# ethereum/c-kzg-4844

Hardware: AMD Instinct MI355X
Metric: blob_to_kzg_commitment throughput (higher is better)
Workload: dtype u32

## Files before the change

### c-kzg-4844_amd/csrc/device.hpp

```cpp
#pragma once
#include <vector>
#include <hip/hip_runtime.h>
#include <atomic>
#include <chrono>
#include <cstdint>
#include <cstdio>
#include <cstdlib>
#include <ctime>
#include <sys/syscall.h>
#include <unistd.h>
#include "g1.hpp"

namespace ckzg {
namespace dev {

constexpr int N_BLOB = 4096;
constexpr int N_EXT = 8192;
constexpr int N_CELL = 64;
constexpr int N_CELLS_EXT = 128;


#ifdef CKZG_AB
static inline long ab_knob(const char *env, long dflt) {
    const char *e = getenv(env);
// ... 93 lines not shown
    for (;;) {
        e = query();
        if (e != hipErrorNotReady) break;
        const int64_t waited = note.waited_us();
        if (waited < spin_us || (waited >= spin_from && waited <= spin_to)) continue;
        if (note.expired()) {
            int d = -1;
            if (hipGetDevice(&d) == hipSuccess && d >= 0 && d < 64) wedged_devices_ref().fetch_or((uint64_t)1 << d, std::memory_order_relaxed);
            (void)hipGetLastError();
            return hipErrorLaunchTimeOut;
        }
        if (div <= 0) continue;
        int64_t step = waited / div;
        step = step < 20 ? 20 : (step > 1000 ? 1000 : step);
        if (waited < spin_from && waited + step > spin_from) step = spin_from - waited;
        sleep_us(step < 5 ? 5 : step);
    }
    last = note.waited_us();
    (void)hipGetLastError();
    return e;
}
inline hipError_t sync_stream(hipStream_t s, int64_t spin_us = 100) {
    return bounded_device_wait([s]() { return hipStreamQuery(s); }, "stream", (const void *)s, spin_us);
}
inline hipError_t sync_event(hipEvent_t ev, int64_t spin_us = 100) {
    return bounded_device_wait([ev]() { return hipEventQuery(ev); }, "event", (const void *)ev, spin_us);
}
inline hipError_t ensure_event(hipEvent_t &e) {
    if (e) return hipSuccess;
    const hipError_t r = hipEventCreateWithFlags(&e, hipEventDisableTiming);
    if (r != hipSuccess) e = nullptr;
    return r;
}

inline std::atomic<int> g_poison_byte{0};
inline int poison_byte() { return g_poison_byte.load(std::memory_order_relaxed); }
inline hipError_t poison_fill(void *p, size_t bytes, hipStream_t s, int byte) {
    if (!p || !bytes) return hipSuccess;
    const hipError_t e = hipMemsetAsync(p, byte, bytes, s);
    return e != hipSuccess ? e : sync_stream(s);
}
inline hipError_t poison_fresh(void *p, size_t bytes, hipStream_t s) {
    const int b = poison_byte();
    return b ? poison_fill(p, bytes, s, b) : hipSuccess;
}

struct FixedBaseTable {
    G1Affine *d_table = nullptr;
    int npoints = 0;
    int wbits = 0;
    int nwin = 0;
    int twin = 0;
    size_t half = 0;
    size_t bytes() const { return (size_t)twin * npoints * half * sizeof(G1Affine); }
    static int twin_for(int wbits) { return 127 / wbits + 1; }
};

struct Scratch {
    void *ptr = nullptr;
    size_t cap = 0;
};

inline double &reserve_scale() {
    static thread_local double s = 1.0;
    return s;
}
struct ReserveScale {
    double old;
    ReserveScale(size_t max_units, size_t n) : old(reserve_scale()) {
        const double f = n ? (double)max_units / (double)n : 1.0;
        reserve_scale() = f < 1.0 ? 1.0 : f;
    }
    ~ReserveScale() { reserve_scale() = old; }
    ReserveScale(const ReserveScale &) = delete;
    ReserveScale &operator=(const ReserveScale &) = delete;
};
inline size_t reserve_scaled(size_t bytes) {
    const double f = reserve_scale();
    if (f <= 1.0) return bytes;
    const double want = (double)bytes * f, cap = (double)bytes + (double)((size_t)1 << 30);
    return (size_t)(want < cap ? want : cap);
}
inline size_t speculative_bytes(size_t need, size_t ahead) {
    if (ahead <= need) return need;
    size_t free_b = 0, total_b = 0;
    if (hipMemGetInfo(&free_b, &total_b) != hipSuccess) {
        (void)hipGetLastError();
        return need;
    }
    return ahead <= free_b / 8 ? ahead : need;
}

struct Arena {
    void *base = nullptr;
    size_t cap = 0, used = 0;
    hipStream_t stream = nullptr;
    bool begin(size_t bytes) {
        bytes += 64 * 256;
        used = 0;
        if (cap >= bytes) return true;
        const size_t old_cap = cap;
        if (base) (void)hipFree(base);
        base = nullptr;
        cap = 0;
        const size_t slack = (bytes >> 1) < ((size_t)256 << 20) ? (bytes >> 1) : ((size_t)256 << 20);
        size_t want = bytes + slack;
// ... 262 lines not shown
```

### c-kzg-4844_amd/csrc/f30_test_ops.hpp

```cpp
#pragma once
#include "g1_30.hpp"

#define CKZG_F30_TEST_OPS                                                                                          \
    OP_MUL(1, 1) OP_MUL(5, 1) OP_MUL(4, 1) OP_MUL(17, 18)                                                          \
    OP_SQR(5) OP_SQR(2) OP_SQR(17)                                                                                 \
    OP_MUL_ADD2(2, 5, 1, 1) OP_MUL_ADD2(17, 17, 5, 5)                                                              \
    OP_NORM(1, 1) OP_NORM(2, 5) OP_NORM(2, 2) OP_NORM(2, 4) OP_NORM(3, 3) OP_NORM(3, 200)                          \
    OP_ADD(1, 1, 1, 1) OP_ADD(1, 1, 2, 2) OP_SUB(1, 1, 1, 4) OP_SUB(1, 1, 1, 3)                                    \
    OP_NEG(1) OP_UNPACK() OP_TO_F28() OP_CONST()

namespace ckzg {
namespace f30test {

constexpr int STATE_WORDS = 52;
constexpr int ENTRY_WORDS = 24;
constexpr int EXIT_WORDS = 56;

template <int L, int V>
HD F30<L, V> ld(const int32_t *p) {
    F30<L, V> r;
#pragma unroll
    for (int j = 0; j < 13; j++) r.l[j] = p[j];
    return r;
}
// ... 45 lines not shown
#undef OP_NEG
#undef OP_UNPACK
#undef OP_TO_F28
#undef OP_CONST
    return false;
}

inline const char *desc() {
    return ""
#define OP_MUL(VA, VB) "mul " #VA " " #VB "\n"
#define OP_SQR(VA) "sqr " #VA "\n"
#define OP_MUL_ADD2(VA, VB, VC, VD) "mul_add2 " #VA " " #VB " " #VC " " #VD "\n"
#define OP_NORM(LA, VA) "norm " #LA " " #VA "\n"
#define OP_ADD(LA, VA, LB, VB) "add " #LA " " #VA " " #LB " " #VB "\n"
#define OP_SUB(LA, VA, LB, VB) "sub " #LA " " #VA " " #LB " " #VB "\n"
#define OP_NEG(V) "neg " #V "\n"
#define OP_UNPACK() "unpack\n"
#define OP_TO_F28() "to_f28\n"
#define OP_CONST() "const\n"
        CKZG_F30_TEST_OPS
#undef OP_MUL
#undef OP_SQR
#undef OP_MUL_ADD2
#undef OP_NORM
#undef OP_ADD
#undef OP_SUB
#undef OP_NEG
#undef OP_UNPACK
#undef OP_TO_F28
#undef OP_CONST
        ;
}

HD void ld_state(XYZZ30 &acc, const int32_t *s) {
    acc.x = ld<1, 4>(s);
    acc.w = ld<1, 1>(s + 13);
    acc.zz = ld<1, 1>(s + 26);
    acc.zzz = ld<1, 1>(s + 39);
}
HD void st_state(int32_t *o, const XYZZ30 &acc) {
#pragma unroll
    for (int j = 0; j < 13; j++) {
        o[j] = acc.x.l[j];
        o[13 + j] = acc.w.l[j];
        o[26 + j] = acc.zz.l[j];
        o[39 + j] = acc.zzz.l[j];
    }
}

HDNI inline void madd_step(int32_t *o, uint8_t *oflags, const int32_t *s, const uint8_t *flags, const uint32_t *entry) {
    XYZZ30 acc;
    ld_state(acc, s);
    bool inf = flags[0] != 0, yneg = flags[1] != 0;
    xyzz30_madd_alt(acc, inf, yneg, f30_unpack(entry), f30_unpack(entry + 12), flags[2] != 0);
    st_state(o, acc);
    oflags[0] = inf ? 1 : 0;
    oflags[1] = yneg ? 1 : 0;
}

HDNI inline void phi_step(int32_t *o, const int32_t *s) {
    XYZZ30 acc;
    ld_state(acc, s);
    xyzz30_apply_phi(acc);
    st_state(o, acc);
}

HDNI inline void exit_step(uint32_t *o, uint8_t *met, const int32_t *s) {
    XYZZ30 acc;
    ld_state(acc, s);
    const XYZZ28 r = xyzz30_to_xyzz28(acc);
#pragma unroll
    for (int j = 0; j < 14; j++) {
        o[j] = r.x.l[j];
        o[14 + j] = r.y.l[j];
        o[28 + j] = r.zz.l[j];
        o[42 + j] = r.zzz.l[j];
    }
    *met = xyzz30_met_equal_x(r) ? 1 : 0;
}

}
}
```

### c-kzg-4844_amd/csrc/fp30.hpp

```cpp
#pragma once
#include "fp28.hpp"

namespace ckzg {

#include "fp30_consts.inc"

template <int LB, int VB>
struct F30 {
    int32_t l[13];
};

HD int32_t f30_sext(uint32_t v) { return (int32_t)(v << 2) >> 2; }

HD void mad64s(int64_t &acc, int32_t a, int32_t b) { acc += (int64_t)a * b; }

HD int32_t f30_take_digit(int64_t &acc, int k) {
    if ((k & 1) != 0) acc += ((int64_t)1 << 29) + ((int64_t)1 << 59);
    const int32_t d = (int32_t)((uint32_t)acc & 0x3fffffffu) - (1 << 29);
    acc >>= 30;
    return d;
}

#if defined(__HIP_DEVICE_COMPILE__) && defined(CKZG_F28_ASM_BLOCKS)
#define CKZG_F30_USE_ASM_BLOCKS 1
#include "fp30_asm_cols.inc"
#endif

namespace f30detail {
constexpr int MAX_TERMS = 31;
}

template <int VA, int VB>
HD F30<1, 1> mul(const F30<1, VA> &a, const F30<1, VB> &b) {
    static_assert(13 + 13 + 2 <= f30detail::MAX_TERMS, "signed 64-bit column accumulator would overflow");
    static_assert(VA * VB <= 314, "Montgomery product would exceed p in magnitude");
#ifdef CKZG_F30_USE_ASM_BLOCKS
    {
        F30<1, 1> ra;
        f30asm_mul(ra.l, a.l, b.l);
        return ra;
    }
#endif
    int32_t q[13];
    int64_t acc = 0;
#pragma unroll
    for (int k = 0; k < 13; k++) {
#pragma unroll
        for (int i = 0; i <= k; i++) mad64s(acc, a.l[i], b.l[k - i]);
#pragma unroll
        for (int i = 0; i < k; i++) mad64s(acc, q[i], F30_P[k - i]);
        q[k] = f30_sext((uint32_t)acc * F30_NINV);
        mad64s(acc, q[k], F30_P[0]);
        acc >>= 30;
    }
    F30<1, 1> r;
#pragma unroll
    for (int k = 13; k < 25; k++) {
#pragma unroll
        for (int i = k - 12; i < 13; i++) mad64s(acc, a.l[i], b.l[k - i]);
#pragma unroll
        for (int i = k - 12; i < 13; i++) mad64s(acc, q[i], F30_P[k - i]);
        r.l[k - 13] = f30_take_digit(acc, k);
    }
    r.l[12] = (int32_t)acc;
    return r;
}

template <int VA, int VB, int VC, int VD>
HD F30<1, 1> mul_add2(const F30<1, VA> &a, const F30<1, VB> &b, const F30<1, VC> &c, const F30<1, VD> &d) {
    static_assert(3 * (F30_SPLIT_LO - 1 + 1) <= f30detail::MAX_TERMS && 3 * (25 - (F30_SPLIT_HI + 1)) <= f30detail::MAX_TERMS,
                  "an unsplit column would overflow");
// ... 74 lines not shown
    return r;
}

template <int LA, int VA, int LB, int VB>
HD F30<LA + LB, VA + VB> add(const F30<LA, VA> &a, const F30<LB, VB> &b) {
    static_assert(LA + LB <= 3, "limb would overflow 32 bits");
    F30<LA + LB, VA + VB> r;
#pragma unroll
    for (int j = 0; j < 13; j++) r.l[j] = a.l[j] + b.l[j];
    return r;
}

template <int LA, int VA, int LB, int VB>
HD F30<LA + LB, VA + VB> sub(const F30<LA, VA> &a, const F30<LB, VB> &b) {
    static_assert(LA + LB <= 3, "limb would overflow 32 bits");
    F30<LA + LB, VA + VB> r;
#pragma unroll
    for (int j = 0; j < 13; j++) r.l[j] = a.l[j] - b.l[j];
    return r;
}

template <int LA, int VA>
HD F30<1, VA> norm(const F30<LA, VA> &a) {
    static_assert(LA <= 3, "limb plus carry would overflow 32 bits");
    static_assert(VA <= 200, "top limb bound");
    F30<1, VA> r;
    int32_t c = 0;
#pragma unroll
    for (int j = 0; j < 12; j++) {
        const int32_t v = a.l[j] + c;
        r.l[j] = f30_sext((uint32_t)v);
        c = LA <= 2 ? (v - r.l[j]) >> 30 : (v >> 30) - (r.l[j] >> 31);
    }
    r.l[12] = a.l[12] + c;
    return r;
}

template <int V>
HD F30<1, V> f30_neg(const F30<1, V> &a) {
    F30<1, V> r;
#pragma unroll
    for (int j = 0; j < 13; j++) r.l[j] = -a.l[j];
    return r;
}

template <int V>
HD F30<1, V> f30_const(const int32_t (&c)[13]) {
    F30<1, V> r;
#pragma unroll
    for (int j = 0; j < 13; j++) r.l[j] = c[j];
    return r;
}

HD F30<1, 1> f30_unpack(const uint32_t *w) {
    F30<1, 1> r;
    uint32_t f[13];
#pragma unroll
    for (int j = 0; j < 13; j++) {
        const int bit = 30 * j, k = bit >> 5, sh = bit & 31;
        uint32_t lo = w[k] >> sh;
        if (sh > 2 && k + 1 < 12) lo |= w[k + 1] << (32 - sh);
        f[j] = lo;
    }
#pragma unroll
    for (int j = 0; j < 13; j++) {
        const int32_t s = j < 12 ? f30_sext(f[j]) : (int32_t)f[j];
        r.l[j] = j == 0 ? s : s + (int32_t)((f[j - 1] >> 29) & 1u);
    }
    return r;
}

HD F28<1, 2> f30_to_f28(const F30<1, 1> &a) {
    uint32_t f[13];
    int32_t c = 0;
#pragma unroll
    for (int j = 0; j < 12; j++) {
        const int32_t v = a.l[j] + F30_P[j] + c;
        f[j] = (uint32_t)v & 0x3fffffffu;
        c = v >> 30;
    }
    f[12] = (uint32_t)(a.l[12] + F30_P[12] + c);
    F28<1, 2> r;
#pragma unroll
    for (int j = 0; j < 14; j++) {
        const int bit = 28 * j, k = bit / 30, sh = bit - 30 * k;
        uint32_t lo = f[k] >> sh;
        if (sh > 2 && k + 1 < 13) lo |= f[k + 1] << (30 - sh);
        r.l[j] = j == 13 ? lo : (lo & M28);
    }
    return r;
}

}
```

### c-kzg-4844_amd/csrc/g1_30.hpp

```cpp
#pragma once
#include "fp30.hpp"
#include "g1_28.hpp"

namespace ckzg {

struct XYZZ30 {
    F30<1, 4> x;
    F30<1, 1> w;
    F30<1, 1> zz;
    F30<1, 1> zzz;
};

template <int V2, int V>
HD F30<1, V2> widen30(const F30<1, V> &a) {
    static_assert(V2 >= V, "bounds can only be loosened");
    F30<1, V2> r;
#pragma unroll
    for (int j = 0; j < 13; j++) r.l[j] = a.l[j];
    return r;
}

HD void xyzz30_madd_alt(XYZZ30 &acc, bool &inf, bool &yneg, const F30<1, 1> &x2, const F30<1, 1> &y2, bool dneg) {
    if (inf) yneg = false;
    const bool tneg = dneg != !yneg;
    const F30<1, 1> ny = f30_neg(y2);
    F30<1, 1> t;
#pragma unroll
    for (int j = 0; j < 13; j++) t.l[j] = tneg ? ny.l[j] : y2.l[j];
    if (inf) {
        acc.x = widen30<4>(mul(x2, f30_const<1>(F30_R392)));
        acc.w = mul(t, f30_const<1>(F30_R394));
        acc.zz = f30_const<1>(F30_R392);
        acc.zzz = f30_const<1>(F30_R394);
        inf = false;
        yneg = true;
        return;
    }
    auto u2 = mul(x2, acc.zz);
    auto tt = mul(t, acc.zzz);
    auto p = norm(sub(u2, acc.x));
    auto r = norm(add(tt, acc.w));
    auto pp = sqr(p);
    auto ppp = mul(p, pp);
    auto q = mul(acc.x, pp);
    auto rr = sqr(r);
    auto t1 = norm(add(ppp, add(q, q)));
    acc.x = norm(sub(rr, t1));
    auto d = norm(sub(q, acc.x));
    acc.w = mul_add2(r, d, acc.w, ppp);
    acc.zz = mul(acc.zz, pp);
    acc.zzz = mul(acc.zzz, ppp);
    yneg = !yneg;
}

HD void xyzz30_apply_phi(XYZZ30 &acc) { acc.x = widen30<4>(mul(acc.x, f30_const<1>(F30_BETA390))); }

HD XYZZ28 xyzz30_to_xyzz28(const XYZZ30 &acc) {
    XYZZ28 o;
    o.x = widen<1, 10>(f30_to_f28(mul(acc.x, f30_const<1>(F30_R392))));
    o.y = widen<1, 6>(f30_to_f28(mul(acc.w, f30_const<1>(F30_R392))));
    o.zz = f30_to_f28(mul(acc.zz, f30_const<1>(F30_R394)));
    o.zzz = f30_to_f28(mul(acc.zzz, f30_const<1>(F30_R394)));
    return o;
}

HD bool xyzz30_met_equal_x(const XYZZ28 &o) { return is_zero(o.zz); }

}
```

### c-kzg-4844_amd/csrc/msm.hip

```cpp
#include <chrono>
#include <cstring>
#include <vector>
#include "device.hpp"
#include "dev_inline.hpp"
#include "g1_28.hpp"
#include "g1_30.hpp"
#include "g1_quad.hpp"

namespace ckzg {
namespace dev {

int scratch_reserve(DeviceCtx *ctx, size_t bytes) {
    if (ctx->scratch.cap >= bytes) return 0;
    const size_t old_cap = ctx->scratch.cap;
    if (ctx->scratch.ptr) {
        HIP_TRY(dev::sync_stream(ctx->stream));
        HIP_TRY(hipFree(ctx->scratch.ptr));
        ctx->scratch.ptr = nullptr;
        ctx->scratch.cap = 0;
    }
    size_t want = bytes + (bytes >> 2);
    if (reserve_scaled(bytes) > want) want = reserve_scaled(bytes);
    if (old_cap) {
        const size_t step = old_cap < ((size_t)2 << 30) ? old_cap : ((size_t)2 << 30);
// ... 230 lines not shown
                tb_store_point(cur[k], x3, y3);
            }
        }
    }
}

int batch_to_affine_device(DeviceCtx *ctx, G1Affine *d_out, const G1XYZZ *d_in, Fp *d_prefix, size_t n) {
    if (n == 0) return 0;
    static const size_t solo_max = (size_t)ab_knob("CKZG_HIP_TO_AFFINE_SOLO_MAX", 4096);
    int L = n >= ((size_t)1 << 20) ? 128 : (n >= ((size_t)1 << 14) ? 16 : (n > solo_max ? 4 : 1));
    size_t threads = (n + L - 1) / L;
    hipLaunchKernelGGL(k_batch_to_affine, dim3((unsigned)((threads + 63) / 64)), dim3(64), 0, ctx->stream,
                       d_out, d_in, d_prefix, n, L, 0);
    HIP_TRY(hipGetLastError());
    return 0;
}


static int enqueue_affine_chain_table(hipStream_t stream, const FixedBaseTable &t, G1Affine *d_table, const G1XYZZ *d_wb,
                                      G1Affine *d_wba, Fp *d_prefix, const std::atomic<bool> *cancel) {
    const size_t nchains = (size_t)t.twin * t.npoints;
    {
        const int Lb = 16;
        const size_t th = (nchains + Lb - 1) / Lb;
        hipLaunchKernelGGL(k_batch_to_affine, dim3((unsigned)((th + 63) / 64)), dim3(64), 0, stream, d_wba, d_wb, d_prefix,
                           nchains, Lb, 1);
    }
    constexpr int LSEG = 8;
    const size_t entries = nchains * t.half;
    size_t seg = entries / ((size_t)262144 * LSEG);
    uint32_t seg2 = 16;
    while (seg2 < 512 && seg2 * 2 <= seg) seg2 *= 2;
    if (seg2 > t.half) seg2 = (uint32_t)t.half;
    const uint32_t nseg = (uint32_t)(t.half / seg2);
    const size_t chains_per_launch = cancel ? (size_t)4 * t.npoints : nchains;
    for (size_t c0 = 0; c0 < nchains; c0 += chains_per_launch) {
        if (cancel && cancel->load(std::memory_order_relaxed)) {
            (void)dev::sync_stream(stream);
            return 5;
        }
        if (cancel && c0) HIP_TRY(dev::sync_stream(stream));
        const size_t nc = nchains - c0 < chains_per_launch ? nchains - c0 : chains_per_launch;
        const size_t units = nc * nseg, threads = (units + LSEG - 1) / LSEG;
        hipLaunchKernelGGL(k_table_seeds, dim3((unsigned)((units + 63) / 64)), dim3(64), 0, stream, d_table + c0 * t.half,
                           d_wba + c0, (uint32_t)nc, (uint32_t)t.half, seg2);
        if (seg2 > 1)
            hipLaunchKernelGGL(k_table_steps<LSEG>, dim3((unsigned)((threads + 63) / 64)), dim3(64), 0, stream,
                               d_table + c0 * t.half, d_wba + c0, (uint32_t)nc, (uint32_t)t.half, seg2);
    }
    HIP_TRY(hipGetLastError());
    return 0;
}

int build_fixed_base_table(DeviceCtx *ctx, FixedBaseTable *t, const G1Affine *d_bases, int npoints,
                           int wbits, double *times_ms, const std::atomic<bool> *cancel) {
    if (wbits < 2 || wbits > 16) return 1;
    const auto t_start = std::chrono::steady_clock::now();
    t->npoints = npoints;
    t->wbits = wbits;
    t->twin = FixedBaseTable::twin_for(wbits);
    t->nwin = 2 * t->twin;
    t->half = (size_t)1 << (wbits - 1);
    DevTmp wb, prefix, table, wba;
    t->d_table = nullptr;
    HIP_TRY(hipMalloc(&table.p, t->bytes()));
    G1Affine *d_table = static_cast<G1Affine *>(table.p);
    HIP_TRY(hipMalloc(&wb.p, (size_t)t->twin * npoints * sizeof(G1XYZZ)));
    HIP_TRY(poison_fresh(wb.p, (size_t)t->twin * npoints * sizeof(G1XYZZ), ctx->stream));
    G1XYZZ *d_wb = static_cast<G1XYZZ *>(wb.p);
    const auto t_alloc = std::chrono::steady_clock::now();
    enqueue_window_bases(ctx->stream, d_wb, d_bases, npoints, wbits, t->twin);
    {
        const size_t nchains = (size_t)t->twin * npoints;
        HIP_TRY(hipMalloc(&wba.p, nchains * sizeof(G1Affine)));
        HIP_TRY(hipMalloc(&prefix.p, nchains * sizeof(Fp)));
        HIP_TRY(poison_fresh(wba.p, nchains * sizeof(G1Affine), ctx->stream));
        HIP_TRY(poison_fresh(prefix.p, nchains * sizeof(Fp), ctx->stream));
        int rc = enqueue_affine_chain_table(ctx->stream, *t, d_table, d_wb, static_cast<G1Affine *>(wba.p),
                                            static_cast<Fp *>(prefix.p), cancel);
        if (rc) return rc;
    }
    HIP_TRY(hipGetLastError());
    HIP_TRY(dev::sync_stream(ctx->stream));
    t->d_table = d_table;
    table.p = nullptr;
    if (times_ms) {
        const auto t_end = std::chrono::steady_clock::now();
        times_ms[0] += std::chrono::duration<double, std::milli>(t_alloc - t_start).count();
        times_ms[1] += std::chrono::duration<double, std::milli>(t_end - t_alloc).count();
    }
    return 0;
}


__global__ void k_blob_digits(int16_t *digits, uint32_t *bad, const uint8_t *blobs, size_t total,
                              int wbits, int twin) {
    size_t gid = blockIdx.x * (size_t)blockDim.x + threadIdx.x;
    if (gid >= total) return;
    size_t blob = gid >> 12;
    uint32_t i = (uint32_t)(gid & 4095);
    uint32_t s[8], r[8];
    load_be256(s, blobs + gid * 32);
#pragma unroll
    for (int k = 0; k < 8; k++) r[k] = FR_R[k];
    if (limbs_geq<8>(s, r)) {
        atomicOr(&bad[blob], 1u);
#pragma unroll
        for (int k = 0; k < 8; k++) s[k] = 0;
    }
    glv_digits(digits + blob * (size_t)(2 * twin) * N_BLOB + i, N_BLOB, s, wbits, twin);
}

__global__ void k_raw_digits(int16_t *digits, const uint32_t *scalars, size_t total, int wbits,
                             int twin) {
    size_t gid = blockIdx.x * (size_t)blockDim.x + threadIdx.x;
    if (gid >= total) return;
    size_t vec = gid >> 12;
    uint32_t i = (uint32_t)(gid & 4095);
    uint32_t s[8];
    const uint4 *q = reinterpret_cast<const uint4 *>(scalars + gid * 8);
    uint4 a = q[0], b = q[1];
    s[0] = a.x; s[1] = a.y; s[2] = a.z; s[3] = a.w;
    s[4] = b.x; s[5] = b.y; s[6] = b.z; s[7] = b.w;
    glv_digits(digits + vec * (size_t)(2 * twin) * N_BLOB + i, N_BLOB, s, wbits, twin);
}



__device__ __forceinline__ void msm_apply_phi(XYZZ28 &acc28) {
    acc28.x = widen<1, 10>(mul(acc28.x, f28_const<1, 1>(FP28_BETA_LAMBDA)));
}
__device__ __forceinline__ void msm_apply_phi(XYZZ30 &acc30) { xyzz30_apply_phi(acc30); }

__device__ __forceinline__ void msm_madd_entry(XYZZ28 &acc, bool &inf, bool &yneg, const uint32_t *wd, bool dneg) {
    xyzz28_madd_alt(acc, inf, yneg, f28_unpack<1>(wd), f28_unpack<1>(wd + 12), dneg);
}
__device__ __forceinline__ void msm_madd_entry(XYZZ30 &acc, bool &inf, bool &yneg, const uint32_t *wd, bool dneg) {
    xyzz30_madd_alt(acc, inf, yneg, f30_unpack(wd), f30_unpack(wd + 12), dneg);
}

__device__ __forceinline__ uint32_t msm_wave_slot_parity() {
    return __builtin_amdgcn_s_getreg(4) & 1u;
}
__device__ __forceinline__ void msm_fair_prio(uint32_t prio_bit, uint32_t parity) {
    if (prio_bit == 0) return;
    const uint32_t slice = (uint32_t)(wall_clock64() >> prio_bit) & 1u;
    if (slice == parity)
        __builtin_amdgcn_s_setprio(2);
    else
        __builtin_amdgcn_s_setprio(0);
}

template <int STRIDE, class ACC>
__device__ __forceinline__ void msm_sum_pairs(ACC &acc28, bool &inf, bool &yneg, const G1Affine *table,
                                              const int16_t *dg, uint32_t first, uint32_t q1, uint32_t phi_pairs,
                                              uint32_t twin, uint32_t ppv, uint32_t npoints, uint32_t voff,
                                              int half_shift, uint32_t prio_bit = 0) {
    bool phi_pending = first < phi_pairs;
    const uint32_t slot_parity = prio_bit ? msm_wave_slot_parity() : 0u;
    uint32_t qn = first;
    int d = 0, d1 = qn < q1 ? dg[qn] : 0;
    uint4 e[6];
#pragma unroll
    for (int k = 0; k < 6; k++) e[k] = make_uint4(0, 0, 0, 0);
    for (; qn < q1 + STRIDE; qn += STRIDE) {
        msm_fair_prio(prio_bit, slot_parity);
        uint4 nx[6];
#pragma unroll
        for (int k = 0; k < 6; k++) nx[k] = make_uint4(0, 0, 0, 0);
        if (d1 != 0) {
            uint32_t w = qn / ppv, i = qn - w * ppv;
            uint32_t tw = w >= twin ? w - twin : w;
            uint32_t mag = (uint32_t)(d1 < 0 ? -d1 : d1);
            const uint4 *src = reinterpret_cast<const uint4 *>(
                table + ((((size_t)tw * npoints + voff + i) << half_shift) + (mag - 1)));
#pragma unroll
            for (int k = 0; k < 6; k++) nx[k] = src[k];
        }
        int d2 = qn + STRIDE < q1 ? dg[qn + STRIDE] : 0;
        if (phi_pending && qn >= phi_pairs + STRIDE) {
            if (!inf) msm_apply_phi(acc28);
            phi_pending = false;
        }
        if (d != 0) {
            uint32_t wd[24];
            uint32_t any = 0;
#pragma unroll
            for (int k = 0; k < 6; k++) {
                wd[4 * k] = e[k].x; wd[4 * k + 1] = e[k].y; wd[4 * k + 2] = e[k].z; wd[4 * k + 3] = e[k].w;
                any |= e[k].x | e[k].y | e[k].z | e[k].w;
            }
            if (any != 0) msm_madd_entry(acc28, inf, yneg, wd, d < 0);
        }
#pragma unroll
        for (int k = 0; k < 6; k++) e[k] = nx[k];
        d = d1;
        d1 = d2;
    }
    if (phi_pending && !inf) msm_apply_phi(acc28);
}

template <int STRIDE>
__device__ __forceinline__ void msm_sum_pairs30(XYZZ30 &acc30, bool &inf, bool &yneg, const G1Affine *table,
                                                const int16_t *dg, uint32_t first, uint32_t q1, uint32_t phi_pairs,
                                                uint32_t twin, uint32_t ppv, uint32_t npoints, uint32_t voff,
                                                int half_shift, uint32_t prio_bit) {
    msm_sum_pairs<STRIDE>(acc30, inf, yneg, table, dg, first, q1, phi_pairs, twin, ppv, npoints, voff, half_shift, prio_bit);
}

#ifdef CKZG_MSM_TRACE
__device__ uint64_t *g_msm_trace = nullptr;
__device__ __forceinline__ void msm_trace_mark(uint32_t wave_slot, int which) {
    if ((threadIdx.x & 63) != 0 || !g_msm_trace) return;
    uint64_t *rec = g_msm_trace + (size_t)wave_slot * 4;
    rec[which] = wall_clock64();
    if (which == 0) {
        rec[2] = __builtin_amdgcn_s_getreg((31 << 11) | 4);
        rec[3] = __builtin_amdgcn_s_getreg((31 << 11) | 20);
    }
}
#endif

template <int THREADS, bool RAW>
__global__ __launch_bounds__(THREADS) void k_msm_accumulate(
    G1XYZZ *partials, const G1Affine *table, const int16_t *digits, uint32_t pairs_per_vec,
    uint32_t pairs_per_block, int half_shift, uint32_t blocks_per_vec, uint32_t ppv,
    uint32_t npoints, uint32_t vecs_per_group, uint32_t part_stride, uint32_t prio_bit) {
    __shared__ uint32_t sh[57][THREADS];
#ifdef CKZG_MSM_TRACE
    msm_trace_mark(blockIdx.x * (THREADS / 64) + threadIdx.x / 64, 0);
#endif
    const uint32_t vec = blockIdx.x / blocks_per_vec, chunk = blockIdx.x % blocks_per_vec;
    const uint32_t q0 = chunk * pairs_per_block;
    const uint32_t q1 = q0 + pairs_per_block < pairs_per_vec ? q0 + pairs_per_block : pairs_per_vec;
    const uint32_t voff = (vec % vecs_per_group) * ppv;
    const uint32_t phi_pairs = pairs_per_vec >> 1, twin = phi_pairs / ppv;
    const int16_t *dg = digits + (size_t)vec * pairs_per_vec;
    XYZZ28 acc28;
    bool inf = true, yneg = false;
#ifdef CKZG_AB
    const bool loop28 = (prio_bit >> 31) != 0;
    prio_bit &= 0x7fffffffu;
#endif
    if constexpr (RAW) {
        msm_sum_pairs<THREADS>(acc28, inf, yneg, table, dg, q0 + threadIdx.x, q1, phi_pairs, twin, ppv, npoints, voff,
                               half_shift, prio_bit);
    } else {
        bool redo = false;
#ifdef CKZG_AB
        redo = loop28;
        if (!loop28)
#endif
        {
            XYZZ30 acc30;
            msm_sum_pairs30<THREADS>(acc30, inf, yneg, table, dg, q0 + threadIdx.x, q1, phi_pairs, twin, ppv, npoints,
                                     voff, half_shift, prio_bit);
            if (!inf) {
                acc28 = xyzz30_to_xyzz28(acc30);
                redo = xyzz30_met_equal_x(acc28);
            }
        }
        if (__syncthreads_or(redo ? 1 : 0)) {
            inf = true, yneg = false;
            msm_sum_pairs<THREADS>(acc28, inf, yneg, table, dg, q0 + threadIdx.x, q1, phi_pairs, twin, ppv, npoints,
                                   voff, half_shift, prio_bit);
        }
    }
    if (prio_bit) __builtin_amdgcn_s_setprio(0);
    xyzz28_fix_sign(acc28, inf, yneg);
    quad::block_reduce_xyzz28_quad<THREADS>(acc28, inf, sh);
    if constexpr (RAW) {
        uint32_t *raw_out = reinterpret_cast<uint32_t *>(partials);
        if (threadIdx.x < 57) raw_out[((size_t)vec * part_stride + chunk) * 57 + threadIdx.x] = sh[threadIdx.x][0];
    } else {
        if (threadIdx.x == 0) partials[(size_t)vec * part_stride + chunk] = xyzz28_to_xyzz(acc28, inf);
    }
#ifdef CKZG_MSM_TRACE
    msm_trace_mark(blockIdx.x * (THREADS / 64) + threadIdx.x / 64, 1);
#endif
}

template <int LPV>
__global__ __launch_bounds__(64) __attribute__((amdgpu_waves_per_eu(2, 2))) void k_msm_small(G1XYZZ *out, const G1Affine *table, const int16_t *digits,
                                                 uint32_t nvec, uint32_t pairs_per_vec, int half_shift,
                                                 uint32_t ppv, uint32_t npoints, uint32_t vecs_per_group, uint32_t prio_bit) {
    __shared__ uint32_t sh[57][LPV == 64 ? 64 : 32];
    constexpr int GROUPS = 64 / LPV;
    const int tid = threadIdx.x, grp = tid / LPV, l = tid % LPV;
    const uint32_t vec = blockIdx.x * GROUPS + grp;
    const uint32_t phi_pairs = pairs_per_vec >> 1, twin = phi_pairs / ppv;
    XYZZ28 acc28;
    bool inf = true, yneg = false;
    if (vec < nvec) {
        const uint32_t voff = (vec % vecs_per_group) * ppv;
        const int16_t *dg = digits + (size_t)vec * pairs_per_vec;
        msm_sum_pairs<LPV>(acc28, inf, yneg, table, dg, (uint32_t)l, pairs_per_vec, phi_pairs, twin, ppv, npoints,
                           voff, half_shift, prio_bit);
    }
    if (prio_bit) __builtin_amdgcn_s_setprio(0);
    xyzz28_fix_sign(acc28, inf, yneg);
    if constexpr (LPV == 64) {
        quad::block_reduce_xyzz28_quad<64>(acc28, inf, sh);
        if (l == 0 && vec < nvec) out[vec] = xyzz28_to_xyzz(acc28, inf);
        return;
    }
    for (int s = LPV / 2; s >= 1; s >>= 1) {
        if (l >= s && l < 2 * s) {
            const uint32_t *src = reinterpret_cast<const uint32_t *>(&acc28);
            const int slot = grp * (LPV / 2) + (l - s);
// ... 175 lines not shown
    static const double TREE = (double)ab_knob("CKZG_HIP_TREE_COST", 9 * 4 * 400 / 2);
    const double ADD = 3542.0;
    const size_t resident = 512;
    uint32_t best_ppb = pairs_per_vec;
    double best = 1e300;
    for (uint32_t bpv = 1; bpv <= 512; bpv++) {
        uint32_t ppb = ((pairs_per_vec + bpv - 1) / bpv + 255) / 256 * 256;
        if (ppb < 512 && bpv > 1) break;
        uint32_t real_bpv = (pairs_per_vec + ppb - 1) / ppb;
        size_t rounds = (nvec * real_bpv + resident - 1) / resident;
        double cost = (double)rounds * ((double)(ppb / 256) * ADD + TREE) + real_bpv * 300.0;
        if (cost < best) {
            best = cost;
            best_ppb = ppb;
        }
    }
    return best_ppb;
}

static uint32_t pick_pairs_per_block_fixed(size_t nvec, uint32_t pairs_per_vec) {
    for (uint32_t ppb = 256; ppb <= 1024; ppb *= 2) {
        const size_t bpv = (pairs_per_vec + ppb - 1) / ppb;
        if (nvec * bpv <= 512 && bpv > 8) return ppb;
    }
    return pick_pairs_per_block(nvec, pairs_per_vec);
}
uint32_t msm_pairs_per_block(size_t nvec, uint32_t pairs_per_vec, bool fixed) {
    return fixed ? pick_pairs_per_block_fixed(nvec, pairs_per_vec) : pick_pairs_per_block(nvec, pairs_per_vec);
}
static size_t partials_bytes(size_t nvec, uint32_t bpv) {
    return bpv > 8 ? nvec * ((size_t)bpv * 57 * sizeof(uint32_t) + sizeof(G1XYZZ)) : nvec * ((size_t)bpv + 1) * sizeof(G1XYZZ);
}

static uint32_t msm_prio_bit() {
    static const uint32_t v = (uint32_t)ab_knob("CKZG_HIP_MSM_PRIO_BIT", 16) |
                              (ab_knob("CKZG_HIP_MSM_LOOP28", 0) ? 0x80000000u : 0u);
    return v;
}
static uint32_t small_prio_bit() {
    static const uint32_t v = (uint32_t)ab_knob("CKZG_HIP_SMALL_PRIO_BIT", 0);
    return v;
}

static int run_msm(DeviceCtx *ctx, const FixedBaseTable &t, uint8_t *d_out48, uint8_t *d_status,
                   const int16_t *d_digits, const uint32_t *d_bad, G1XYZZ *d_partials, size_t nvec,
                   uint32_t ppb) {
    uint32_t pairs_per_vec = (uint32_t)t.nwin * t.npoints;
    uint32_t bpv = (pairs_per_vec + ppb - 1) / ppb;
    HIP_TRY(hipEventRecord(ctx->ev[2], ctx->stream));
    if (bpv > 8 && bpv <= 512 && ppb <= 1024 && nvec * bpv <= 512) {
        uint32_t *d_raw = reinterpret_cast<uint32_t *>(d_partials);
        hipLaunchKernelGGL((k_msm_accumulate<256, true>), dim3((unsigned)(nvec * bpv)), dim3(256), 0, ctx->stream,
                           d_partials, t.d_table, d_digits, pairs_per_vec, ppb, t.wbits - 1, bpv,
                           (uint32_t)t.npoints, (uint32_t)t.npoints, 1u, bpv, msm_prio_bit());
        HIP_TRY(hipEventRecord(ctx->ev[3], ctx->stream));
        hipLaunchKernelGGL(k_msm_fold_finalize, dim3((unsigned)nvec), dim3(FOLD_THREADS), 0, ctx->stream, d_out48, d_status, d_raw,
                           d_bad, bpv);
        HIP_TRY(hipEventRecord(ctx->ev[4], ctx->stream));
        HIP_TRY(hipGetLastError());
        return 0;
    }
    hipLaunchKernelGGL((k_msm_accumulate<256, false>), dim3((unsigned)(nvec * bpv)), dim3(256), 0, ctx->stream,
                       d_partials, t.d_table, d_digits, pairs_per_vec, ppb, t.wbits - 1, bpv,
                       (uint32_t)t.npoints, (uint32_t)t.npoints, 1u, bpv, msm_prio_bit());
    HIP_TRY(hipEventRecord(ctx->ev[3], ctx->stream));
    if (bpv > 8) {
        G1XYZZ *d_sums = d_partials + nvec * (size_t)bpv;
        hipLaunchKernelGGL(k_msm_reduce_partials, dim3((unsigned)nvec), dim3(64), 0, ctx->stream, d_sums,
                           d_partials, bpv);
        hipLaunchKernelGGL(k_msm_finalize, dim3((unsigned)((nvec + 63) / 64)), dim3(64), 0, ctx->stream,
                           d_out48, d_status, d_sums, d_bad, 1u, nvec);
    } else if (bpv >= 2 && nvec <= 4096) {
        if (bpv <= 2)
            hipLaunchKernelGGL(k_msm_finalize_tree<2>, dim3((unsigned)((nvec + 31) / 32)), dim3(64), 0, ctx->stream, d_out48,
                               d_status, d_partials, d_bad, bpv, nvec);
        else if (bpv <= 4)
            hipLaunchKernelGGL(k_msm_finalize_tree<4>, dim3((unsigned)((nvec + 15) / 16)), dim3(64), 0, ctx->stream, d_out48,
                               d_status, d_partials, d_bad, bpv, nvec);
        else
            hipLaunchKernelGGL(k_msm_finalize_tree<8>, dim3((unsigned)((nvec + 7) / 8)), dim3(64), 0, ctx->stream, d_out48,
                               d_status, d_partials, d_bad, bpv, nvec);
    } else {
        hipLaunchKernelGGL(k_msm_finalize, dim3((unsigned)((nvec + 63) / 64)), dim3(64), 0, ctx->stream,
                           d_out48, d_status, d_partials, d_bad, bpv, nvec);
    }
    HIP_TRY(hipEventRecord(ctx->ev[4], ctx->stream));
    HIP_TRY(hipGetLastError());
    return 0;
}

static size_t align_up(size_t v, size_t a) { return (v + a - 1) / a * a; }

void commit_collect_times(DeviceCtx *ctx) {
    float ms;
#ifdef CKZG_FOLD_TRACE
    {
        uint64_t h[16] = {};
        if (hipMemcpyFromSymbol(h, HIP_SYMBOL(g_fold_trace), sizeof h) == hipSuccess && getenv("CKZG_FOLD_TRACE_PRINT"))
            fprintf(stderr, "[fold trace, 10 ns ticks] level0 %llu  tree %llu  inv(extra) %llu  to_affine %llu  compress %llu  store %llu\n",
                    (unsigned long long)(h[1] - h[0]), (unsigned long long)(h[2] - h[1]), (unsigned long long)(h[3] - h[2]),
                    (unsigned long long)(h[4] - h[3]), (unsigned long long)(h[5] - h[4]), (unsigned long long)(h[6] - h[5]));
    }
#endif
    if (hipEventElapsedTime(&ms, ctx->ev[1], ctx->ev[2]) == hipSuccess) ctx->last_ms[0] = ms;
    if (hipEventElapsedTime(&ms, ctx->ev[2], ctx->ev[3]) == hipSuccess) ctx->last_ms[1] = ms;
    if (hipEventElapsedTime(&ms, ctx->ev[3], ctx->ev[4]) == hipSuccess) ctx->last_ms[2] = ms;
    if (hipEventElapsedTime(&ms, ctx->ev[1], ctx->ev[4]) == hipSuccess) ctx->last_ms[3] = ms;
    (void)hipGetLastError();
}

int msm_small_vectors_device(DeviceCtx *ctx, const FixedBaseTable &t, G1XYZZ *d_out,
                             const int16_t *d_digits, size_t nvec, uint32_t ppv,
                             uint32_t vecs_per_group) {
    if (nvec == 0) return 0;
    uint32_t pairs_per_vec = (uint32_t)t.nwin * ppv;
    HIP_TRY(hipEventRecord(ctx->ev[5], ctx->stream));
    static const long forced_lpv = ab_knob("CKZG_HIP_SMALL_LPV", 0);
// ... 100 lines not shown
int commit_one_graph_build(DeviceCtx *ctx, hipGraphExec_t *exec_out, uint8_t *d_out48, uint8_t *d_status,
                           const uint8_t *d_blob, const void *h_in, void *h_res) {
    const FixedBaseTable &t = ctx->commit;
    if (!t.d_table) return 2;
    const size_t n = 1;
    uint32_t pairs_per_vec = (uint32_t)t.nwin * t.npoints;
    uint32_t ppb = pick_pairs_per_block_fixed(n, pairs_per_vec);
    uint32_t bpv = (pairs_per_vec + ppb - 1) / ppb;
    if (!(bpv > 8 && bpv <= 512 && ppb <= 1024 && n * bpv <= 512)) return 4;
    size_t dig_bytes = align_up(n * (size_t)pairs_per_vec * sizeof(int16_t), 256);
    size_t bad_bytes = align_up(n * sizeof(uint32_t), 256);
    if (ctx->scratch.cap < dig_bytes + bad_bytes + align_up(partials_bytes(n, bpv), 256)) return 2;
    uint8_t *base = static_cast<uint8_t *>(ctx->scratch.ptr);
    int16_t *d_digits = reinterpret_cast<int16_t *>(base);
    uint32_t *d_bad = reinterpret_cast<uint32_t *>(base + dig_bytes);
    G1XYZZ *d_partials = reinterpret_cast<G1XYZZ *>(base + dig_bytes + bad_bytes);
    const uint32_t *d_raw = reinterpret_cast<const uint32_t *>(d_partials);

    struct GraphOwner {
        hipGraph_t g = nullptr;
        ~GraphOwner() {
            if (g) (void)hipGraphDestroy(g);
        }
    } own;
    HIP_TRY(hipGraphCreate(&own.g, 0));
    hipGraphNode_t n_in, n_zero, n_digits, n_acc, n_fold, n_out;
    HIP_TRY(hipGraphAddMemcpyNode1D(&n_in, own.g, nullptr, 0, const_cast<uint8_t *>(d_blob), h_in, (size_t)N_BLOB * 32,
                                    hipMemcpyHostToDevice));
    hipMemsetParams zp;
    memset(&zp, 0, sizeof zp);
    zp.dst = d_bad;
    zp.elementSize = 4;
    zp.width = n;
    zp.height = 1;
    zp.pitch = n * 4;
    zp.value = 0;
    HIP_TRY(hipGraphAddMemsetNode(&n_zero, own.g, &n_in, 1, &zp));

    hipKernelNodeParams kp;
    size_t total = n * N_BLOB;
    int wbits = t.wbits, twin = t.twin;
    const uint8_t *blob_arg = d_blob;
    void *a_digits[] = {&d_digits, &d_bad, &blob_arg, &total, &wbits, &twin};
    memset(&kp, 0, sizeof kp);
    kp.func = reinterpret_cast<void *>(k_blob_digits);
    kp.gridDim = dim3((unsigned)((total + 255) / 256));
    kp.blockDim = dim3(256);
    kp.kernelParams = a_digits;
    HIP_TRY(hipGraphAddKernelNode(&n_digits, own.g, &n_zero, 1, &kp));

    const G1Affine *table = t.d_table;
    const int16_t *digits_arg = d_digits;
    int half_shift = t.wbits - 1;
    uint32_t npts = (uint32_t)t.npoints, one = 1u, prio = msm_prio_bit();
    void *a_acc[] = {&d_partials, &table, &digits_arg, &pairs_per_vec, &ppb, &half_shift, &bpv, &npts, &npts, &one, &bpv, &prio};
    memset(&kp, 0, sizeof kp);
    kp.func = reinterpret_cast<void *>(k_msm_accumulate<256, true>);
    kp.gridDim = dim3((unsigned)(n * bpv));
    kp.blockDim = dim3(256);
    kp.kernelParams = a_acc;
    HIP_TRY(hipGraphAddKernelNode(&n_acc, own.g, &n_digits, 1, &kp));

    const uint32_t *bad_arg = d_bad;
    void *a_fold[] = {&d_out48, &d_status, &d_raw, &bad_arg, &bpv};
    memset(&kp, 0, sizeof kp);
    kp.func = reinterpret_cast<void *>(k_msm_fold_finalize);
    kp.gridDim = dim3((unsigned)n);
    kp.blockDim = dim3(FOLD_THREADS);
    kp.kernelParams = a_fold;
    HIP_TRY(hipGraphAddKernelNode(&n_fold, own.g, &n_acc, 1, &kp));

    HIP_TRY(hipGraphAddMemcpyNode1D(&n_out, own.g, &n_fold, 1, h_res, d_out48, n * 49, hipMemcpyDeviceToHost));
    hipGraphExec_t exec = nullptr;
    HIP_TRY(hipGraphInstantiate(&exec, own.g, nullptr, nullptr, 0));
    *exec_out = exec;
    return 0;
}

int commit_accumulate8_enqueue(DeviceCtx *ctx, G1XYZZ *d_part8, uint32_t *d_bad, const uint8_t *d_blobs, size_t k) {
    if (k == 0) return 0;
    const FixedBaseTable &t = ctx->commit;
    if (!t.d_table) return 2;
    uint32_t pairs_per_vec = (uint32_t)t.nwin * t.npoints;
    uint32_t ppb = pick_pairs_per_block(k, pairs_per_vec);
    uint32_t bpv = (pairs_per_vec + ppb - 1) / ppb;
    if (bpv > 8) return 4;
    size_t dig_bytes = align_up(k * (size_t)pairs_per_vec * sizeof(int16_t), 256);
    if (ctx->scratch.cap < dig_bytes) return 2;
    int16_t *d_digits = reinterpret_cast<int16_t *>(ctx->scratch.ptr);
    size_t total = k * N_BLOB;
    hipLaunchKernelGGL(k_blob_digits, dim3((unsigned)((total + 255) / 256)), dim3(256), 0, ctx->stream,
                       d_digits, d_bad, d_blobs, total, t.wbits, t.twin);
    hipLaunchKernelGGL((k_msm_accumulate<256, false>), dim3((unsigned)(k * bpv)), dim3(256), 0, ctx->stream,
                       d_part8, t.d_table, d_digits, pairs_per_vec, ppb, t.wbits - 1, bpv,
                       (uint32_t)t.npoints, (uint32_t)t.npoints, 1u, 8u, msm_prio_bit());
    HIP_TRY(hipGetLastError());
    return 0;
}

bool commit_chunk_fits8(const DeviceCtx *ctx, size_t k) {
    const FixedBaseTable &t = ctx->commit;
    uint32_t pairs_per_vec = (uint32_t)t.nwin * t.npoints;
    uint32_t ppb = pick_pairs_per_block(k, pairs_per_vec);
    return (pairs_per_vec + ppb - 1) / ppb <= 8;
}

int commit_finalize8_enqueue(DeviceCtx *ctx, uint8_t *d_out48, uint8_t *d_status, const G1XYZZ *d_part8,
                             const uint32_t *d_bad, size_t n) {
    if (n == 0) return 0;
    if (n <= 4096)
        hipLaunchKernelGGL(k_msm_finalize_tree<8>, dim3((unsigned)((n + 7) / 8)), dim3(64), 0, ctx->stream, d_out48, d_status,
                           d_part8, d_bad, 8u, n);
    else
        hipLaunchKernelGGL(k_msm_finalize, dim3((unsigned)((n + 63) / 64)), dim3(64), 0, ctx->stream, d_out48, d_status,
                           d_part8, d_bad, 8u, n);
    HIP_TRY(hipGetLastError());
    return 0;
}

int commit_blobs_device(DeviceCtx *ctx, uint8_t *d_out48, uint8_t *d_status, const uint8_t *d_blobs,
                        size_t n) {
    if (n == 0) return 0;
    int rc = scratch_reserve(ctx, commit_scratch_bytes(ctx, n));
    if (rc) return rc;
#ifdef CKZG_MSM_TRACE
    const char *trace_file = getenv("CKZG_HIP_MSM_TRACE_FILE");
    uint64_t *d_trace = nullptr;
    size_t trace_waves = 0;
    if (trace_file && *trace_file) {
        const FixedBaseTable &t = ctx->commit;
        uint32_t ppv = (uint32_t)t.nwin * t.npoints, ppb = pick_pairs_per_block_fixed(n, ppv);
        trace_waves = n * ((ppv + ppb - 1) / ppb) * 4;
        HIP_TRY(hipMalloc(&d_trace, trace_waves * 32));
        HIP_TRY(hipMemset(d_trace, 0, trace_waves * 32));
        HIP_TRY(hipMemcpyToSymbol(HIP_SYMBOL(g_msm_trace), &d_trace, sizeof d_trace));
    }
#endif
    rc = commit_blobs_enqueue(ctx, d_out48, d_status, d_blobs, n);
    if (rc) return rc;
    HIP_TRY(dev::sync_stream(ctx->stream));
    commit_collect_times(ctx);
#ifdef CKZG_MSM_TRACE
    if (d_trace) {
        std::vector<uint64_t> h(trace_waves * 4);
        HIP_TRY(hipMemcpy(h.data(), d_trace, trace_waves * 32, hipMemcpyDeviceToHost));
        uint64_t *null_ptr = nullptr;
        HIP_TRY(hipMemcpyToSymbol(HIP_SYMBOL(g_msm_trace), &null_ptr, sizeof null_ptr));
        (void)hipFree(d_trace);
// ... 205 lines not shown
```

Measured before the change: 104,800.

## Fold y-negation into F30 unpack and specialize the 30-bit MSM inner loop

Negation of the table point's y coordinate is folded into f30_unpack as a ones-complement plus one, replacing a separate f30_neg and a 13-limb select. The 30-bit MSM pair loop gets its own dedicated implementation: it loads table entries one step ahead, computes the entry address incrementally when the window stride is uniform, and skips the all-zero entry check when table construction found no point at infinity among the bases. A small kernel and a host readback during table build set the new has_inf flag. This trims per-step ALU work in the hot accumulate loop, at the cost of more code paths and a changed digit-extraction routine.

New measurement: 104,400 (median of 2 runs). Within noise of the previous version (-0.4%).

```diff
diff --git a/c-kzg-4844_amd/csrc/device.hpp b/c-kzg-4844_amd/csrc/device.hpp
--- a/c-kzg-4844_amd/csrc/device.hpp
+++ b/c-kzg-4844_amd/csrc/device.hpp
@@ -169,6 +169,7 @@
     int nwin = 0;
     int twin = 0;
     size_t half = 0;
+    bool has_inf = true;
     size_t bytes() const { return (size_t)twin * npoints * half * sizeof(G1Affine); }
     static int twin_for(int wbits) { return 127 / wbits + 1; }
 };
diff --git a/c-kzg-4844_amd/csrc/f30_test_ops.hpp b/c-kzg-4844_amd/csrc/f30_test_ops.hpp
--- a/c-kzg-4844_amd/csrc/f30_test_ops.hpp
+++ b/c-kzg-4844_amd/csrc/f30_test_ops.hpp
@@ -121,7 +121,7 @@
     XYZZ30 acc;
     ld_state(acc, s);
     bool inf = flags[0] != 0, yneg = flags[1] != 0;
-    xyzz30_madd_alt(acc, inf, yneg, f30_unpack(entry), f30_unpack(entry + 12), flags[2] != 0);
+    xyzz30_madd_packed(acc, inf, yneg, entry, flags[2] != 0);
     st_state(o, acc);
     oflags[0] = inf ? 1 : 0;
     oflags[1] = yneg ? 1 : 0;
diff --git a/c-kzg-4844_amd/csrc/fp30.hpp b/c-kzg-4844_amd/csrc/fp30.hpp
--- a/c-kzg-4844_amd/csrc/fp30.hpp
+++ b/c-kzg-4844_amd/csrc/fp30.hpp
@@ -15,8 +15,13 @@
 HD void mad64s(int64_t &acc, int32_t a, int32_t b) { acc += (int64_t)a * b; }
 
 HD int32_t f30_take_digit(int64_t &acc, int k) {
-    if ((k & 1) != 0) acc += ((int64_t)1 << 29) + ((int64_t)1 << 59);
-    const int32_t d = (int32_t)((uint32_t)acc & 0x3fffffffu) - (1 << 29);
+    int32_t d;
+    if ((k & 1) != 0) {
+        d = f30_sext((uint32_t)acc);
+        acc += ((int64_t)1 << 29) + ((int64_t)1 << 59);
+    } else {
+        d = (int32_t)((uint32_t)acc & 0x3fffffffu) - (1 << 29);
+    }
     acc >>= 30;
     return d;
 }
@@ -197,20 +202,23 @@
     return r;
 }
 
-HD F30<1, 1> f30_unpack(const uint32_t *w) {
-    F30<1, 1> r;
-    uint32_t f[13];
+HD F30<1, 1> f30_unpack(const uint32_t *w, bool neg = false) {
+    const uint32_t one = neg ? 1u : 0u, m = 0u - one;
+    F30<1, 1> r;
+    uint32_t v[12], f[13];
+#pragma unroll
+    for (int k = 0; k < 12; k++) v[k] = w[k] ^ m;
 #pragma unroll
     for (int j = 0; j < 13; j++) {
         const int bit = 30 * j, k = bit >> 5, sh = bit & 31;
-        uint32_t lo = w[k] >> sh;
-        if (sh > 2 && k + 1 < 12) lo |= w[k + 1] << (32 - sh);
+        uint32_t lo = j < 12 ? v[k] >> sh : (uint32_t)((int32_t)v[k] >> sh);
+        if (sh > 2 && k + 1 < 12) lo |= v[k + 1] << (32 - sh);
         f[j] = lo;
     }
 #pragma unroll
     for (int j = 0; j < 13; j++) {
         const int32_t s = j < 12 ? f30_sext(f[j]) : (int32_t)f[j];
-        r.l[j] = j == 0 ? s : s + (int32_t)((f[j - 1] >> 29) & 1u);
+        r.l[j] = j == 0 ? s + (int32_t)one : s + (int32_t)((f[j - 1] >> 29) & 1u);
     }
     return r;
 }
diff --git a/c-kzg-4844_amd/csrc/g1_30.hpp b/c-kzg-4844_amd/csrc/g1_30.hpp
--- a/c-kzg-4844_amd/csrc/g1_30.hpp
+++ b/c-kzg-4844_amd/csrc/g1_30.hpp
@@ -20,13 +20,12 @@
     return r;
 }
 
-HD void xyzz30_madd_alt(XYZZ30 &acc, bool &inf, bool &yneg, const F30<1, 1> &x2, const F30<1, 1> &y2, bool dneg) {
+HD bool xyzz30_entry_tneg(bool inf, bool &yneg, bool dneg) {
     if (inf) yneg = false;
-    const bool tneg = dneg != !yneg;
-    const F30<1, 1> ny = f30_neg(y2);
-    F30<1, 1> t;
-#pragma unroll
-    for (int j = 0; j < 13; j++) t.l[j] = tneg ? ny.l[j] : y2.l[j];
+    return dneg != !yneg;
+}
+
+HD void xyzz30_madd_signed(XYZZ30 &acc, bool &inf, bool &yneg, const F30<1, 1> &x2, const F30<1, 1> &t) {
     if (inf) {
         acc.x = widen30<4>(mul(x2, f30_const<1>(F30_R392)));
         acc.w = mul(t, f30_const<1>(F30_R394));
@@ -53,6 +52,20 @@
     yneg = !yneg;
 }
 
+HD void xyzz30_madd_alt(XYZZ30 &acc, bool &inf, bool &yneg, const F30<1, 1> &x2, const F30<1, 1> &y2, bool dneg) {
+    const bool tneg = xyzz30_entry_tneg(inf, yneg, dneg);
+    const F30<1, 1> ny = f30_neg(y2);
+    F30<1, 1> t;
+#pragma unroll
+    for (int j = 0; j < 13; j++) t.l[j] = tneg ? ny.l[j] : y2.l[j];
+    xyzz30_madd_signed(acc, inf, yneg, x2, t);
+}
+
+HD void xyzz30_madd_packed(XYZZ30 &acc, bool &inf, bool &yneg, const uint32_t *wd, bool dneg) {
+    const bool tneg = xyzz30_entry_tneg(inf, yneg, dneg);
+    xyzz30_madd_signed(acc, inf, yneg, f30_unpack(wd), f30_unpack(wd + 12, tneg));
+}
+
 HD void xyzz30_apply_phi(XYZZ30 &acc) { acc.x = widen30<4>(mul(acc.x, f30_const<1>(F30_BETA390))); }
 
 HD XYZZ28 xyzz30_to_xyzz28(const XYZZ30 &acc) {
diff --git a/c-kzg-4844_amd/csrc/msm.hip b/c-kzg-4844_amd/csrc/msm.hip
--- a/c-kzg-4844_amd/csrc/msm.hip
+++ b/c-kzg-4844_amd/csrc/msm.hip
@@ -306,6 +306,11 @@
     return 0;
 }
 
+__global__ void k_any_base_inf(uint32_t *flag, const G1Affine *bases, int npoints) {
+    const int i = blockIdx.x * blockDim.x + threadIdx.x;
+    if (i < npoints && bases[i].is_inf()) atomicOr(flag, 1u);
+}
+
 int build_fixed_base_table(DeviceCtx *ctx, FixedBaseTable *t, const G1Affine *d_bases, int npoints,
                            int wbits, double *times_ms, const std::atomic<bool> *cancel) {
     if (wbits < 2 || wbits > 16) return 1;
@@ -315,8 +320,13 @@
     t->twin = FixedBaseTable::twin_for(wbits);
     t->nwin = 2 * t->twin;
     t->half = (size_t)1 << (wbits - 1);
-    DevTmp wb, prefix, table, wba;
+    DevTmp wb, prefix, table, wba, any_inf;
     t->d_table = nullptr;
+    t->has_inf = true;
+    HIP_TRY(hipMalloc(&any_inf.p, sizeof(uint32_t)));
+    HIP_TRY(hipMemsetAsync(any_inf.p, 0, sizeof(uint32_t), ctx->stream));
+    hipLaunchKernelGGL(k_any_base_inf, dim3((unsigned)((npoints + 255) / 256)), dim3(256), 0, ctx->stream,
+                       static_cast<uint32_t *>(any_inf.p), d_bases, npoints);
     HIP_TRY(hipMalloc(&table.p, t->bytes()));
     G1Affine *d_table = static_cast<G1Affine *>(table.p);
     HIP_TRY(hipMalloc(&wb.p, (size_t)t->twin * npoints * sizeof(G1XYZZ)));
@@ -335,7 +345,10 @@
         if (rc) return rc;
     }
     HIP_TRY(hipGetLastError());
+    uint32_t h_any_inf = 1;
+    HIP_TRY(hipMemcpyAsync(&h_any_inf, any_inf.p, sizeof h_any_inf, hipMemcpyDeviceToHost, ctx->stream));
     HIP_TRY(dev::sync_stream(ctx->stream));
+    t->has_inf = h_any_inf != 0;
     t->d_table = d_table;
     table.p = nullptr;
     if (times_ms) {
@@ -384,13 +397,9 @@
 __device__ __forceinline__ void msm_apply_phi(XYZZ28 &acc28) {
     acc28.x = widen<1, 10>(mul(acc28.x, f28_const<1, 1>(FP28_BETA_LAMBDA)));
 }
-__device__ __forceinline__ void msm_apply_phi(XYZZ30 &acc30) { xyzz30_apply_phi(acc30); }
 
 __device__ __forceinline__ void msm_madd_entry(XYZZ28 &acc, bool &inf, bool &yneg, const uint32_t *wd, bool dneg) {
     xyzz28_madd_alt(acc, inf, yneg, f28_unpack<1>(wd), f28_unpack<1>(wd + 12), dneg);
-}
-__device__ __forceinline__ void msm_madd_entry(XYZZ30 &acc, bool &inf, bool &yneg, const uint32_t *wd, bool dneg) {
-    xyzz30_madd_alt(acc, inf, yneg, f30_unpack(wd), f30_unpack(wd + 12), dneg);
 }
 
 __device__ __forceinline__ uint32_t msm_wave_slot_parity() {
@@ -405,8 +414,8 @@
         __builtin_amdgcn_s_setprio(0);
 }
 
-template <int STRIDE, class ACC>
-__device__ __forceinline__ void msm_sum_pairs(ACC &acc28, bool &inf, bool &yneg, const G1Affine *table,
+template <int STRIDE>
+__device__ __forceinline__ void msm_sum_pairs(XYZZ28 &acc28, bool &inf, bool &yneg, const G1Affine *table,
                                               const int16_t *dg, uint32_t first, uint32_t q1, uint32_t phi_pairs,
                                               uint32_t twin, uint32_t ppv, uint32_t npoints, uint32_t voff,
                                               int half_shift, uint32_t prio_bit = 0) {
@@ -456,10 +465,60 @@
 
 template <int STRIDE>
 __device__ __forceinline__ void msm_sum_pairs30(XYZZ30 &acc30, bool &inf, bool &yneg, const G1Affine *table,
-                                                const int16_t *dg, uint32_t first, uint32_t q1, uint32_t phi_pairs,
-                                                uint32_t twin, uint32_t ppv, uint32_t npoints, uint32_t voff,
-                                                int half_shift, uint32_t prio_bit) {
-    msm_sum_pairs<STRIDE>(acc30, inf, yneg, table, dg, first, q1, phi_pairs, twin, ppv, npoints, voff, half_shift, prio_bit);
+                                                const int16_t *dg, uint32_t q0, uint32_t lane, uint32_t q1,
+                                                uint32_t phi_pairs, uint32_t twin, uint32_t ppv, uint32_t npoints,
+                                                uint32_t voff, int half_shift, uint32_t prio_bit, bool table_inf) {
+    const bool uniform_w = ppv % STRIDE == 0 && q0 % STRIDE == 0;
+    bool phi_pending = q0 + lane < phi_pairs;
+    const uint32_t slot_parity = prio_bit ? msm_wave_slot_parity() : 0u;
+    const uint32_t lane_off = (lane << half_shift) - 1;
+    uint32_t w = q0 / ppv, i = q0 - w * ppv;
+    int d = 0, d1 = q0 + lane < q1 ? dg[q0 + lane] : 0;
+    uint4 e[6];
+#pragma unroll
+    for (int k = 0; k < 6; k++) e[k] = make_uint4(0, 0, 0, 0);
+    for (uint32_t uq = q0; uq < q1 + STRIDE; uq += STRIDE) {
+        const uint32_t qn = uq + lane;
+        msm_fair_prio(prio_bit, slot_parity);
+        if (phi_pending && qn >= phi_pairs + STRIDE) {
+            if (!inf) xyzz30_apply_phi(acc30);
+            phi_pending = false;
+        }
+        uint32_t wd[24];
+#pragma unroll
+        for (int k = 0; k < 6; k++) {
+            wd[4 * k] = e[k].x; wd[4 * k + 1] = e[k].y; wd[4 * k + 2] = e[k].z; wd[4 * k + 3] = e[k].w;
+        }
+        bool add = d != 0;
+        if (table_inf) {
+            uint32_t any = 0;
+#pragma unroll
+            for (int k = 0; k < 24; k++) any |= wd[k];
+            add = add && any != 0;
+        }
+        const bool tneg = xyzz30_entry_tneg(inf, yneg, d < 0);
+        const F30<1, 1> x2 = f30_unpack(wd), t = f30_unpack(wd + 12, tneg);
+        const uint32_t mag = (uint32_t)(d1 < 0 ? -d1 : d1);
+        const G1Affine *entry = table;
+        if (uniform_w) {
+            const uint32_t wt = w >= twin ? w - twin : w, tw = wt < twin ? wt : twin - 1;
+            entry = table + (((size_t)tw * npoints + voff + i) << half_shift) + (lane_off + (mag > 1 ? mag : 1u));
+            i += STRIDE;
+            if (i >= ppv) i = 0, w++;
+        } else if (d1 != 0) {
+            uint32_t wl = qn / ppv, il = qn - wl * ppv;
+            uint32_t tw = wl >= twin ? wl - twin : wl;
+            entry = table + ((((size_t)tw * npoints + voff + il) << half_shift) + (mag - 1));
+        }
+        const uint4 *src = reinterpret_cast<const uint4 *>(entry);
+#pragma unroll
+        for (int k = 0; k < 6; k++) e[k] = src[k];
+        int d2 = qn + STRIDE < q1 ? dg[qn + STRIDE] : 0;
+        if (add) xyzz30_madd_signed(acc30, inf, yneg, x2, t);
+        d = d1;
+        d1 = d2;
+    }
+    if (phi_pending && !inf) xyzz30_apply_phi(acc30);
 }
 
 #ifdef CKZG_MSM_TRACE
@@ -479,7 +538,7 @@
 __global__ __launch_bounds__(THREADS) void k_msm_accumulate(
     G1XYZZ *partials, const G1Affine *table, const int16_t *digits, uint32_t pairs_per_vec,
     uint32_t pairs_per_block, int half_shift, uint32_t blocks_per_vec, uint32_t ppv,
-    uint32_t npoints, uint32_t vecs_per_group, uint32_t part_stride, uint32_t prio_bit) {
+    uint32_t npoints, uint32_t vecs_per_group, uint32_t part_stride, uint32_t prio_bit, uint32_t table_inf) {
     __shared__ uint32_t sh[57][THREADS];
 #ifdef CKZG_MSM_TRACE
     msm_trace_mark(blockIdx.x * (THREADS / 64) + threadIdx.x / 64, 0);
@@ -507,8 +566,8 @@
 #endif
         {
             XYZZ30 acc30;
-            msm_sum_pairs30<THREADS>(acc30, inf, yneg, table, dg, q0 + threadIdx.x, q1, phi_pairs, twin, ppv, npoints,
-                                     voff, half_shift, prio_bit);
+            msm_sum_pairs30<THREADS>(acc30, inf, yneg, table, dg, q0, threadIdx.x, q1, phi_pairs, twin, ppv, npoints,
+                                     voff, half_shift, prio_bit, table_inf != 0);
             if (!inf) {
                 acc28 = xyzz30_to_xyzz28(acc30);
                 redo = xyzz30_met_equal_x(acc28);
@@ -790,7 +849,7 @@
         uint32_t *d_raw = reinterpret_cast<uint32_t *>(d_partials);
         hipLaunchKernelGGL((k_msm_accumulate<256, true>), dim3((unsigned)(nvec * bpv)), dim3(256), 0, ctx->stream,
                            d_partials, t.d_table, d_digits, pairs_per_vec, ppb, t.wbits - 1, bpv,
-                           (uint32_t)t.npoints, (uint32_t)t.npoints, 1u, bpv, msm_prio_bit());
+                           (uint32_t)t.npoints, (uint32_t)t.npoints, 1u, bpv, msm_prio_bit(), t.has_inf ? 1u : 0u);
         HIP_TRY(hipEventRecord(ctx->ev[3], ctx->stream));
         hipLaunchKernelGGL(k_msm_fold_finalize, dim3((unsigned)nvec), dim3(FOLD_THREADS), 0, ctx->stream, d_out48, d_status, d_raw,
                            d_bad, bpv);
@@ -800,7 +859,7 @@
     }
     hipLaunchKernelGGL((k_msm_accumulate<256, false>), dim3((unsigned)(nvec * bpv)), dim3(256), 0, ctx->stream,
                        d_partials, t.d_table, d_digits, pairs_per_vec, ppb, t.wbits - 1, bpv,
-                       (uint32_t)t.npoints, (uint32_t)t.npoints, 1u, bpv, msm_prio_bit());
+                       (uint32_t)t.npoints, (uint32_t)t.npoints, 1u, bpv, msm_prio_bit(), t.has_inf ? 1u : 0u);
     HIP_TRY(hipEventRecord(ctx->ev[3], ctx->stream));
     if (bpv > 8) {
         G1XYZZ *d_sums = d_partials + nvec * (size_t)bpv;
@@ -1007,8 +1066,9 @@
     const G1Affine *table = t.d_table;
     const int16_t *digits_arg = d_digits;
     int half_shift = t.wbits - 1;
-    uint32_t npts = (uint32_t)t.npoints, one = 1u, prio = msm_prio_bit();
-    void *a_acc[] = {&d_partials, &table, &digits_arg, &pairs_per_vec, &ppb, &half_shift, &bpv, &npts, &npts, &one, &bpv, &prio};
+    uint32_t npts = (uint32_t)t.npoints, one = 1u, prio = msm_prio_bit(), table_inf = t.has_inf ? 1u : 0u;
+    void *a_acc[] = {&d_partials, &table, &digits_arg, &pairs_per_vec, &ppb, &half_shift, &bpv, &npts, &npts, &one, &bpv, &prio,
+                     &table_inf};
     memset(&kp, 0, sizeof kp);
     kp.func = reinterpret_cast<void *>(k_msm_accumulate<256, true>);
     kp.gridDim = dim3((unsigned)(n * bpv));
@@ -1048,7 +1108,7 @@
                        d_digits, d_bad, d_blobs, total, t.wbits, t.twin);
     hipLaunchKernelGGL((k_msm_accumulate<256, false>), dim3((unsigned)(k * bpv)), dim3(256), 0, ctx->stream,
                        d_part8, t.d_table, d_digits, pairs_per_vec, ppb, t.wbits - 1, bpv,
-                       (uint32_t)t.npoints, (uint32_t)t.npoints, 1u, 8u, msm_prio_bit());
+                       (uint32_t)t.npoints, (uint32_t)t.npoints, 1u, 8u, msm_prio_bit(), t.has_inf ? 1u : 0u);
     HIP_TRY(hipGetLastError());
     return 0;
 }
```
